# myscience/open-genie

Measured on NVIDIA B200. Metric: videotokenizer_train_step_frames_per_sec, higher is better.
Workload: dtype bf16

## Files before the change

open_genie_b200/csrc/conv3d_wgrad.cu:

```cuda
#include <stdlib.h>

#include "og_host.cuh"
#include "og_ptx.cuh"

namespace og {
extern std::atomic<uint64_t> g_launches;

struct WgradParams {
  int kt, kh, kw, pt, ph, pw;
  int ntaps, taps_per_group, num_groups, splitk;
  int block_n;
  int bw_log2, bh_log2, bt_log2, bn_log2;
  int tiles_w, tiles_h, tiles_t;
  int num_ksteps;
  int cin, cout;
  float* dw;
  long long ld_dw;
  int a_stages, b_stages;
  int sx_t, sx_h, sx_w;
  int vec_ok;
  float* dbias;
  int n_bias;
  int bias_col;
  int plain_store;
  int dbg;
};

static constexpr int kWThreads = 192;
static constexpr int kVox = 64;
static constexpr int kPanelBytes = kVox * 128;
static constexpr int kWABytes = 2 * kPanelBytes;
static constexpr int kWMaxStages = 12;

__global__ void __launch_bounds__(kWThreads, 1)
    og_conv_wgrad_kernel(const __grid_constant__ CUtensorMap mapDY, const __grid_constant__ CUtensorMap mapX,
                         const WgradParams p) {
  extern __shared__ uint8_t smem_raw[];
  uint8_t* smem = reinterpret_cast<uint8_t*>((reinterpret_cast<uintptr_t>(smem_raw) + 1023) & ~uintptr_t(1023));
  const int tap_bytes = (p.block_n / 64) * kPanelBytes;
  const int b_bytes = 2 * tap_bytes;
  uint8_t* smem_a = smem;
  uint8_t* smem_b = smem + p.a_stages * kWABytes;
  uint8_t* smem_ones = smem_b + p.b_stages * b_bytes;
  uint64_t* bars = reinterpret_cast<uint64_t*>(smem_ones + 2048);
  uint64_t* full_a = bars;
  uint64_t* empty_a = bars + kWMaxStages;
  uint64_t* full_b = bars + 2 * kWMaxStages;
  uint64_t* empty_b = bars + 3 * kWMaxStages;
  uint64_t* tmem_full = bars + 4 * kWMaxStages;
  uint32_t* tmem_slot = reinterpret_cast<uint32_t*>(bars + 4 * kWMaxStages + 1);

  const int warp = warp_idx_uniform();
  const int lane = threadIdx.x & 31;
  const int co0 = blockIdx.x * 128;
  const int ci0 = blockIdx.y * p.block_n;
  const int split = blockIdx.z / p.num_groups;
  const int group = blockIdx.z - split * p.num_groups;
  const int tap0 = group * p.taps_per_group;
  const int ntap = min(p.taps_per_group, p.ntaps - tap0);
  const bool do_bias = p.dbias != nullptr && blockIdx.y == 0 && group == p.num_groups - 1;
  const int ks_begin = (int)(((long long)p.num_ksteps * split) / p.splitk);
  const int ks_end = (int)(((long long)p.num_ksteps * (split + 1)) / p.splitk);

  if (warp == 0 && lane == 0) {
    tma_prefetch_desc(&mapDY);
    tma_prefetch_desc(&mapX);
    for (int s = 0; s < p.a_stages; ++s) {
      mbar_init(&full_a[s], 1);
      mbar_init(&empty_a[s], 1);
    }
    for (int s = 0; s < p.b_stages; ++s) {
      mbar_init(&full_b[s], 1);
      mbar_init(&empty_b[s], 1);
    }
    mbar_init(tmem_full, 1);
    fence_mbar_init();
  }
  if (warp == 1) tmem_alloc(tmem_slot, 512);
  if (do_bias) {
    for (int i = threadIdx.x; i < 2048 / 4; i += kWThreads) reinterpret_cast<uint32_t*>(smem_ones)[i] = 0x3F803F80u;
    fence_proxy_async_smem();
  }
  tc_fence_before();
  __syncthreads();
  tc_fence_after();
  const uint32_t tmem_base = *tmem_slot;

  if (warp == 0) {
    {
      int sa = 0, sb = 0;
      uint32_t pha = 0, phb = 0;
      int off_w[4], off_h[4], off_t[4];
#pragma unroll
      for (int j = 0; j < 4; ++j) {
        const int tap = tap0 + (j < ntap ? j : 0);
        off_t[j] = tap / (p.kh * p.kw) - p.pt;
        off_h[j] = (tap / p.kw) % p.kh - p.ph;
        off_w[j] = tap % p.kw - p.pw;
      }
      const int per_sample = p.tiles_w * p.tiles_h * p.tiles_t;
      int tn = ks_begin / per_sample;
      int r = ks_begin - tn * per_sample;
      int tw = r % p.tiles_w;
      r /= p.tiles_w;
      int th = r % p.tiles_h;
      int tt = r / p.tiles_h;
      const int panels = p.block_n / 64;
      for (int ks = ks_begin; ks < ks_end; ++ks) {
        const int n = tn << p.bn_log2, w0 = tw << p.bw_log2, h0 = th << p.bh_log2, t0 = tt << p.bt_log2;
        mbar_wait(&empty_a[sa], pha ^ 1);
        if (elect_one()) {
          mbar_expect_tx(&full_a[sa], kWABytes);
          tma_load_5d(smem_a + sa * kWABytes, &mapDY, &full_a[sa], co0, w0, h0, t0, n);
          tma_load_5d(smem_a + sa * kWABytes + kPanelBytes, &mapDY, &full_a[sa], co0 + 64, w0, h0, t0, n);
        }
        __syncwarp();
        if (++sa == p.a_stages) {
          sa = 0;
          pha ^= 1;
        }
#pragma unroll
        for (int j = 0; j < 4; j += 2) {
          if (j < ntap) {
            const int nt = (ntap - j) < 2 ? 1 : 2;
            mbar_wait(&empty_b[sb], phb ^ 1);
            if (elect_one()) {
              mbar_expect_tx(&full_b[sb], (uint32_t)(nt * tap_bytes));
              uint8_t* dst = smem_b + sb * b_bytes;
#pragma unroll
              for (int u = 0; u < 2; ++u) {
                if (u < nt) {
                  for (int pp = 0; pp < panels; ++pp)
                    tma_load_5d(dst + u * tap_bytes + pp * kPanelBytes, &mapX, &full_b[sb], ci0 + pp * 64,
                                w0 * p.sx_w + off_w[j + u], h0 * p.sx_h + off_h[j + u], t0 * p.sx_t + off_t[j + u], n);
                }
              }
            }
            __syncwarp();
            if (++sb == p.b_stages) {
              sb = 0;
              phb ^= 1;
            }
          }
        }
        if (++tw == p.tiles_w) {
          tw = 0;
          if (++th == p.tiles_h) {
            th = 0;
            if (++tt == p.tiles_t) {
              tt = 0;
              ++tn;
            }
          }
        }
      }
    }
    __syncwarp();
  } else if (warp == 1) {
    {
      const uint32_t amn = (p.dbg & 1) ? 0u : 1u, bmn = (p.dbg & 2) ? 0u : 1u;
      const uint32_t idesc1 = umma_idesc_bf16(128, (uint32_t)p.block_n, amn, bmn);
      const uint32_t idesc2 = umma_idesc_bf16(128, (uint32_t)(2 * p.block_n), amn, bmn);
      const uint32_t idesc_ones = umma_idesc_bf16(128, 16u, amn, 1u);
      int sa = 0, sb = 0;
      uint32_t pha = 0, phb = 0;
      for (int ks = ks_begin; ks < ks_end; ++ks) {
        mbar_wait(&full_a[sa], pha);
        tc_fence_after();
        const uint32_t a_addr = smem_u32(smem_a + sa * kWABytes);
        for (int j = 0; j < ntap; j += 2) {
          mbar_wait(&full_b[sb], phb);
          tc_fence_after();
          const uint32_t b_addr = smem_u32(smem_b + sb * b_bytes);
          const uint32_t d_tmem = tmem_base + j * p.block_n;
          const uint32_t idesc = (ntap - j >= 2) ? idesc2 : idesc1;
          if (elect_one()) {
#pragma unroll
            for (int k = 0; k < kVox / 16; ++k) {
              const uint64_t adesc = umma_smem_desc_sw128(a_addr + k * 2048, kPanelBytes, 1024);
              const uint64_t bdesc = umma_smem_desc_sw128(b_addr + k * 2048, kPanelBytes, 1024);
              umma_bf16_ss(d_tmem, adesc, bdesc, idesc, (ks > ks_begin || k > 0) ? 1u : 0u);
            }
            umma_commit(&empty_b[sb]);
          }
          __syncwarp();
          if (++sb == p.b_stages) {
            sb = 0;
            phb ^= 1;
          }
        }
        if (do_bias && elect_one()) {
          const uint32_t ones_addr = smem_u32(smem_ones);
#pragma unroll
          for (int k = 0; k < kVox / 16; ++k)
            umma_bf16_ss(tmem_base + p.bias_col, umma_smem_desc_sw128(a_addr + k * 2048, kPanelBytes, 1024),
                         umma_smem_desc_sw128(ones_addr, kPanelBytes, 1024), idesc_ones, (ks > ks_begin || k > 0) ? 1u : 0u);
        }
        __syncwarp();
        if (elect_one()) umma_commit(&empty_a[sa]);
        __syncwarp();
        if (++sa == p.a_stages) {
          sa = 0;
          pha ^= 1;
        }
      }
      if (elect_one()) umma_commit(tmem_full);
    }
    __syncwarp();
  } else {
    const int q = warp & 3;
    const int co = co0 + q * 32 + lane;
    if (p.dbg & 8)
      mbar_wait(tmem_full, 0);
    else
      mbar_wait_relaxed(tmem_full, 0);
    tc_fence_after();
    for (int j = 0; j < ntap && !(p.dbg & 4); ++j) {
      const int tap = tap0 + j;
      for (int c = 0; c < p.block_n; c += 32) {
        uint32_t v[32];
        tmem_ld_32x32(tmem_base + j * p.block_n + c + ((uint32_t)(q * 32) << 16), v);
        tmem_ld_wait();
        if (co < p.cout) {
          float* dst = p.dw + (long long)co * p.ld_dw + (long long)tap * p.cin + ci0 + c;
          if (p.vec_ok && ci0 + c + 32 <= p.cin && p.splitk == 1 && p.plain_store) {
#pragma unroll
            for (int jj = 0; jj < 32; jj += 4)
              *reinterpret_cast<float4*>(dst + jj) = make_float4(__uint_as_float(v[jj]), __uint_as_float(v[jj + 1]),
                                                                 __uint_as_float(v[jj + 2]), __uint_as_float(v[jj + 3]));
          } else if (p.vec_ok && ci0 + c + 32 <= p.cin) {
#pragma unroll
            for (int jj = 0; jj < 32; jj += 4)
              asm volatile("red.global.add.v4.f32 [%0], {%1, %2, %3, %4};" ::"l"(dst + jj), "f"(__uint_as_float(v[jj])),
                           "f"(__uint_as_float(v[jj + 1])), "f"(__uint_as_float(v[jj + 2])),
                           "f"(__uint_as_float(v[jj + 3]))
                           : "memory");
          } else {
#pragma unroll
            for (int jj = 0; jj < 32; ++jj)
              if (ci0 + c + jj < p.cin) atomicAdd(dst + jj, __uint_as_float(v[jj]));
          }
        }
      }
    }
    if (do_bias) {
      uint32_t v[16];
      tmem_ld_32x16(tmem_base + p.bias_col + ((uint32_t)(q * 32) << 16), v);
      tmem_ld_wait();
      if (co < p.n_bias) atomicAdd(p.dbias + co, __uint_as_float(v[0]));
    }
    tc_fence_before();
  }

  tc_fence_before();
  __syncthreads();
  if (warp == 1) {
    tc_fence_after();
    tmem_dealloc(tmem_base, 512);
  }
}

}

static int launch_wgrad(const void* dy, int cout, const void* x, int cin, float* dw, int64_t ld_dw, int kt, int kh, int kw,
                        int pt, int ph, int pw, int N, int T, int H, int W, int Ti, int Hi, int Wi, int st, int sh, int sw,
                        og_stream_t stream, float* dbias = nullptr, int n_bias = 0) {
  using namespace og;
  OG_REQUIRE(dy && x && dw, "conv3d_wgrad: null pointer");
  OG_REQUIRE(!dbias || (n_bias > 0 && n_bias <= cout), "conv3d_wgrad: n_bias=%d must be in 1..cout", n_bias);
  OG_REQUIRE(cin > 0 && cin % 64 == 0, "conv3d_wgrad: cin=%d must be a multiple of 64", cin);
  OG_REQUIRE(cout > 0 && cout % 8 == 0, "conv3d_wgrad: cout=%d must be a multiple of 8 (TMA row stride)", cout);
  OG_REQUIRE(kt >= 1 && kh >= 1 && kw >= 1 && pt >= 0 && ph >= 0 && pw >= 0 && pt < kt && ph < kh && pw < kw,
             "conv3d_wgrad: bad kernel/padding");
  OG_REQUIRE(st >= 1 && sh >= 1 && sw >= 1 && st <= 8 && sh <= 8 && sw <= 8, "conv3d_wgrad: bad stride");
  int bw, bh, bt, bn;
  choose_voxel_box(kVox, N, T, H, W, &bw, &bh, &bt, &bn);
  WgradParams p;
  memset(&p, 0, sizeof(p));
  p.kt = kt; p.kh = kh; p.kw = kw; p.pt = pt; p.ph = ph; p.pw = pw;
  p.sx_t = st; p.sx_h = sh; p.sx_w = sw;
  p.ntaps = kt * kh * kw;
  p.block_n = (cin % 128 == 0) ? 128 : 64;
  p.taps_per_group = 512 / p.block_n;
  if (p.taps_per_group > 4) p.taps_per_group = 4;
  if (p.taps_per_group > p.ntaps) p.taps_per_group = p.ntaps;
  p.num_groups = (p.ntaps + p.taps_per_group - 1) / p.taps_per_group;
  p.bw_log2 = ilog2(bw); p.bh_log2 = ilog2(bh); p.bt_log2 = ilog2(bt); p.bn_log2 = ilog2(bn);
  p.tiles_w = (W + bw - 1) / bw; p.tiles_h = (H + bh - 1) / bh; p.tiles_t = (T + bt - 1) / bt;
  p.num_ksteps = ((N + bn - 1) / bn) * p.tiles_w * p.tiles_h * p.tiles_t;
  p.cin = cin; p.cout = cout; p.dw = dw; p.ld_dw = ld_dw;
  const int co_tiles = (cout + 127) / 128;
  const int ci_tiles = cin / p.block_n;
  const int base_ctas = co_tiles * ci_tiles * p.num_groups;
  const int sms = num_sms();
  int max_split = p.num_ksteps / 4;
  if (max_split < 1) max_split = 1;
  if (max_split > 128) max_split = 128;
  int splitk = 1;
  double best = -1.0;
  for (int s = 1; s <= max_split; ++s) {
    const long long total = (long long)base_ctas * s;
    const long long waves = (total + sms - 1) / sms;
    if (waves > 3 && s > 1) break;
    const double eff = (double)total / (double)(waves * sms);
    if (eff > best + 1e-9) {
      best = eff;
      splitk = s;
    }
  }
  p.splitk = splitk;
  {
    const char* e = getenv("OG_WGRAD_DBG");
    p.dbg = e ? atoi(e) : 0;
    const char* ps = getenv("OG_WGRAD_PLAIN_STORE");
    p.plain_store = ps ? atoi(ps) : 0;
  }
  p.vec_ok = (ld_dw % 4 == 0) && (cin % 4 == 0) && ((reinterpret_cast<uintptr_t>(dw) & 15) == 0);
  bool colsum_after = false;
  if (dbias) {
    const int ntap_last = p.ntaps - (p.num_groups - 1) * p.taps_per_group;
    if (ntap_last * p.block_n + 16 <= 512 && !(p.dbg & 3)) {
      p.dbias = dbias;
      p.n_bias = n_bias;
      p.bias_col = ntap_last * p.block_n;
    } else {
      colsum_after = true;
    }
  }
  const int b_bytes = 2 * (p.block_n / 64) * kPanelBytes;
  p.a_stages = 3;
  p.b_stages = (int)((216 * 1024 - p.a_stages * kWABytes) / b_bytes);
  if (p.b_stages > kWMaxStages) p.b_stages = kWMaxStages;
  const size_t smem_bytes = (size_t)p.a_stages * kWABytes + (size_t)p.b_stages * b_bytes + 2048  + 1024 + 512;

  CUtensorMap mapDY, mapX;
  {
    uint64_t dims[5] = {(uint64_t)cout, (uint64_t)W, (uint64_t)H, (uint64_t)T, (uint64_t)N};
    uint64_t str[4] = {(uint64_t)cout * 2, (uint64_t)W * cout * 2, (uint64_t)H * W * cout * 2,
                       (uint64_t)T * H * W * cout * 2};
    uint32_t box[5] = {64, (uint32_t)bw, (uint32_t)bh, (uint32_t)bt, (uint32_t)bn};
    int r = make_tmap_bf16(&mapDY, dy, 5, dims, str, box);
    if (r != OG_OK) return r;
  }
  {
    uint64_t dims[5] = {(uint64_t)cin, (uint64_t)Wi, (uint64_t)Hi, (uint64_t)Ti, (uint64_t)N};
    uint64_t str[4] = {(uint64_t)cin * 2, (uint64_t)Wi * cin * 2, (uint64_t)Hi * Wi * cin * 2,
                       (uint64_t)Ti * Hi * Wi * cin * 2};
    uint32_t box[5] = {64, (uint32_t)(bw * sw), (uint32_t)(bh * sh), (uint32_t)(bt * st), (uint32_t)bn};
    uint32_t es[5] = {1, (uint32_t)sw, (uint32_t)sh, (uint32_t)st, 1};
    OG_REQUIRE(box[1] <= 256 && box[2] <= 256 && box[3] <= 256, "conv3d_wgrad: strided box exceeds the TMA limit");
    int r = make_tmap_bf16(&mapX, x, 5, dims, str, box, es);
    if (r != OG_OK) return r;
  }
  static bool attr_set = false;
  if (!attr_set) {
    OG_CHECK_CUDA(cudaFuncSetAttribute(og_conv_wgrad_kernel, cudaFuncAttributeMaxDynamicSharedMemorySize, 227 * 1024));
    attr_set = true;
  }
  dim3 grid(co_tiles, ci_tiles, p.num_groups * p.splitk);
  og_conv_wgrad_kernel<<<grid, kWThreads, smem_bytes, (cudaStream_t)stream>>>(mapDY, mapX, p);
  OG_CHECK_CUDA(cudaGetLastError());
  g_launches.fetch_add(1);
  if (colsum_after) return og_colsum(dy, (int64_t)N * T * H * W, n_bias, cout, dbias, stream);
  return OG_OK;
}

extern "C" int og_conv3d_wgrad(const void* dy, int cout, const void* x, int cin, float* dw, int64_t ld_dw, int kt,
                               int kh, int kw, int pt, int ph, int pw, int N, int T, int H, int W,
                               og_stream_t stream) {
  return launch_wgrad(dy, cout, x, cin, dw, ld_dw, kt, kh, kw, pt, ph, pw, N, T, H, W, T, H, W, 1, 1, 1, stream);
}

extern "C" int og_conv3d_wgrad_bias(const void* dy, int cout, const void* x, int cin, float* dw, int64_t ld_dw, int kt,
                                    int kh, int kw, int pt, int ph, int pw, int N, int T, int H, int W, float* dbias,
                                    int n_bias, og_stream_t stream) {
  if (!dbias) {
    og::set_error("conv3d_wgrad_bias: dbias is NULL");
    return OG_ERR_INVALID_ARGUMENT;
  }
  return launch_wgrad(dy, cout, x, cin, dw, ld_dw, kt, kh, kw, pt, ph, pw, N, T, H, W, T, H, W, 1, 1, 1, stream, dbias, n_bias);
}

extern "C" int og_conv3d_strided_wgrad(const void* dy, int cout, const void* x, int cin, float* dw, int64_t ld_dw, int kt,
                                       int kh, int kw, int st, int sh, int sw, int pt, int ph, int pw, int N, int T, int H,
                                       int W, og_stream_t stream) {
  const int To = (T + pt - kt) / st + 1, Ho = (H + 2 * ph - kh) / sh + 1, Wo = (W + 2 * pw - kw) / sw + 1;
  if (To < 1 || Ho < 1 || Wo < 1) {
    og::set_error("conv3d_strided_wgrad: empty output");
    return OG_ERR_INVALID_ARGUMENT;
  }
  return launch_wgrad(dy, cout, x, cin, dw, ld_dw, kt, kh, kw, pt, ph, pw, N, To, Ho, Wo, T, H, W, st, sh, sw, stream);
}
```

open_genie_b200/csrc/og_ptx.cuh:

```cuda
#pragma once
#include <cuda.h>
#include <cuda_bf16.h>
#include <cuda_runtime.h>
#include <stdint.h>

namespace og {

__device__ __forceinline__ uint32_t smem_u32(const void* p) {
  return static_cast<uint32_t>(__cvta_generic_to_shared(p));
}

__device__ __forceinline__ int warp_idx_uniform() { return __shfl_sync(0xffffffffu, (int)(threadIdx.x >> 5), 0); }
__device__ __forceinline__ bool elect_one() {
  uint32_t pred;
  asm volatile(
      "{\n"
      ".reg .pred P1;\n"
      "elect.sync _|P1, 0xffffffff;\n"
      "selp.u32 %0, 1, 0, P1;\n"
      "}\n"
      : "=r"(pred));
  return pred != 0;
}

__device__ __forceinline__ void mbar_init(uint64_t* bar, uint32_t count) {
  asm volatile("mbarrier.init.shared::cta.b64 [%0], %1;" ::"r"(smem_u32(bar)), "r"(count) : "memory");
}
__device__ __forceinline__ void fence_mbar_init() {
  asm volatile("fence.mbarrier_init.release.cluster;" ::: "memory");
}
__device__ __forceinline__ void fence_proxy_async_smem() {
  asm volatile("fence.proxy.async.shared::cta;" ::: "memory");
}
__device__ __forceinline__ void mbar_expect_tx(uint64_t* bar, uint32_t bytes) {
  asm volatile("mbarrier.arrive.expect_tx.shared::cta.b64 _, [%0], %1;" ::"r"(smem_u32(bar)), "r"(bytes)
               : "memory");
}
__device__ __forceinline__ void mbar_arrive(uint64_t* bar) {
  asm volatile("mbarrier.arrive.shared::cta.b64 _, [%0];" ::"r"(smem_u32(bar)) : "memory");
}
__device__ __forceinline__ bool mbar_try_wait(uint64_t* bar, uint32_t parity) {
  uint32_t ok;
  asm volatile(
      "{\n\t.reg .pred p;\n\t"
      "mbarrier.try_wait.parity.shared::cta.b64 p, [%1], %2;\n\t"
      "selp.u32 %0, 1, 0, p;\n\t}"
      : "=r"(ok)
      : "r"(smem_u32(bar)), "r"(parity)
      : "memory");
  return ok != 0;
}
#ifndef OG_MBAR_SPIN_LIMIT
#define OG_MBAR_SPIN_LIMIT (1u << 24)
#endif
__device__ __forceinline__ void mbar_wait(uint64_t* bar, uint32_t parity) {
  uint32_t spins = 0;
  while (!mbar_try_wait(bar, parity)) {
    if (++spins > OG_MBAR_SPIN_LIMIT) {
      printf("og: mbarrier wait timed out (block %d,%d,%d thread %d)\n", blockIdx.x, blockIdx.y, blockIdx.z,
             threadIdx.x);
      __trap();
    }
  }
}

__device__ __forceinline__ void mbar_wait_relaxed(uint64_t* bar, uint32_t parity) {
  uint32_t spins = 0;
  while (!mbar_try_wait(bar, parity)) {
    __nanosleep(spins < 64 ? 64 : 512);
    if (++spins > (OG_MBAR_SPIN_LIMIT >> 2)) {
      printf("og: mbarrier (relaxed) wait timed out (block %d,%d,%d thread %d)\n", blockIdx.x, blockIdx.y, blockIdx.z,
             threadIdx.x);
      __trap();
    }
  }
}

__device__ __forceinline__ void tma_prefetch_desc(const CUtensorMap* map) {
  asm volatile("prefetch.tensormap [%0];" ::"l"(map) : "memory");
}
__device__ __forceinline__ void tma_load_2d(void* smem, const CUtensorMap* map, uint64_t* bar, int c0, int c1) {
  asm volatile(
      "cp.async.bulk.tensor.2d.shared::cluster.global.mbarrier::complete_tx::bytes [%0], [%1, {%3, %4}], [%2];" ::"r"(
          smem_u32(smem)),
      "l"(map), "r"(smem_u32(bar)), "r"(c0), "r"(c1)
      : "memory");
}
__device__ __forceinline__ void tma_load_3d(void* smem, const CUtensorMap* map, uint64_t* bar, int c0, int c1, int c2) {
  asm volatile(
      "cp.async.bulk.tensor.3d.shared::cluster.global.mbarrier::complete_tx::bytes [%0], [%1, {%3, %4, %5}], "
      "[%2];" ::"r"(smem_u32(smem)),
      "l"(map), "r"(smem_u32(bar)), "r"(c0), "r"(c1), "r"(c2)
      : "memory");
}
__device__ __forceinline__ void tma_load_4d(void* smem, const CUtensorMap* map, uint64_t* bar, int c0, int c1, int c2,
                                            int c3) {
  asm volatile(
      "cp.async.bulk.tensor.4d.shared::cluster.global.mbarrier::complete_tx::bytes [%0], [%1, {%3, %4, %5, %6}], "
      "[%2];" ::"r"(smem_u32(smem)),
      "l"(map), "r"(smem_u32(bar)), "r"(c0), "r"(c1), "r"(c2), "r"(c3)
      : "memory");
}
__device__ __forceinline__ void tma_load_5d(void* smem, const CUtensorMap* map, uint64_t* bar, int c0, int c1, int c2,
                                            int c3, int c4) {
  asm volatile(
      "cp.async.bulk.tensor.5d.shared::cluster.global.mbarrier::complete_tx::bytes [%0], [%1, {%3, %4, %5, %6, %7}], "
      "[%2];" ::"r"(smem_u32(smem)),
      "l"(map), "r"(smem_u32(bar)), "r"(c0), "r"(c1), "r"(c2), "r"(c3), "r"(c4)
      : "memory");
}

__device__ __forceinline__ void tmem_alloc(uint32_t* smem_result, uint32_t ncols) {
  asm volatile("tcgen05.alloc.cta_group::1.sync.aligned.shared::cta.b32 [%0], %1;" ::"r"(smem_u32(smem_result)),
               "r"(ncols)
               : "memory");
  asm volatile("tcgen05.relinquish_alloc_permit.cta_group::1.sync.aligned;" ::: "memory");
}
__device__ __forceinline__ void tmem_dealloc(uint32_t taddr, uint32_t ncols) {
  asm volatile("tcgen05.dealloc.cta_group::1.sync.aligned.b32 %0, %1;" ::"r"(taddr), "r"(ncols) : "memory");
}
__device__ __forceinline__ void tc_fence_before() { asm volatile("tcgen05.fence::before_thread_sync;" ::: "memory"); }
__device__ __forceinline__ void tc_fence_after() { asm volatile("tcgen05.fence::after_thread_sync;" ::: "memory"); }

__device__ __forceinline__ void umma_bf16_ss(uint32_t tmem_d, uint64_t adesc, uint64_t bdesc, uint32_t idesc,
                                             uint32_t accumulate) {
  asm volatile(
      "{\n\t.reg .pred p;\n\t"
      "setp.ne.b32 p, %4, 0;\n\t"
      "tcgen05.mma.cta_group::1.kind::f16 [%0], %1, %2, %3, p;\n\t}" ::"r"(tmem_d),
      "l"(adesc), "l"(bdesc), "r"(idesc), "r"(accumulate)
      : "memory");
}
__device__ __forceinline__ void umma_commit(uint64_t* bar) {
  asm volatile("tcgen05.commit.cta_group::1.mbarrier::arrive::one.shared::cluster.b64 [%0];" ::"r"(smem_u32(bar))
               : "memory");
}
__device__ __forceinline__ void tmem_ld_wait() { asm volatile("tcgen05.wait::ld.sync.aligned;" ::: "memory"); }

__device__ __forceinline__ void tmem_ld_32x32(uint32_t taddr, uint32_t (&v)[32]) {
  asm volatile(
      "tcgen05.ld.sync.aligned.32x32b.x32.b32 "
      "{%0, %1, %2, %3, %4, %5, %6, %7, %8, %9, %10, %11, %12, %13, %14, %15, "
      "%16, %17, %18, %19, %20, %21, %22, %23, %24, %25, %26, %27, %28, %29, %30, %31}, [%32];"
      : "=r"(v[0]), "=r"(v[1]), "=r"(v[2]), "=r"(v[3]), "=r"(v[4]), "=r"(v[5]), "=r"(v[6]), "=r"(v[7]), "=r"(v[8]),
        "=r"(v[9]), "=r"(v[10]), "=r"(v[11]), "=r"(v[12]), "=r"(v[13]), "=r"(v[14]), "=r"(v[15]), "=r"(v[16]),
        "=r"(v[17]), "=r"(v[18]), "=r"(v[19]), "=r"(v[20]), "=r"(v[21]), "=r"(v[22]), "=r"(v[23]), "=r"(v[24]),
        "=r"(v[25]), "=r"(v[26]), "=r"(v[27]), "=r"(v[28]), "=r"(v[29]), "=r"(v[30]), "=r"(v[31])
      : "r"(taddr)
      : "memory");
}
__device__ __forceinline__ void tmem_st_32x32(uint32_t taddr, const uint32_t (&v)[32]) {
  asm volatile(
      "tcgen05.st.sync.aligned.32x32b.x32.b32 [%0], "
      "{%1, %2, %3, %4, %5, %6, %7, %8, %9, %10, %11, %12, %13, %14, %15, %16, "
      "%17, %18, %19, %20, %21, %22, %23, %24, %25, %26, %27, %28, %29, %30, %31, %32};" ::"r"(taddr),
      "r"(v[0]), "r"(v[1]), "r"(v[2]), "r"(v[3]), "r"(v[4]), "r"(v[5]), "r"(v[6]), "r"(v[7]), "r"(v[8]), "r"(v[9]),
      "r"(v[10]), "r"(v[11]), "r"(v[12]), "r"(v[13]), "r"(v[14]), "r"(v[15]), "r"(v[16]), "r"(v[17]), "r"(v[18]),
      "r"(v[19]), "r"(v[20]), "r"(v[21]), "r"(v[22]), "r"(v[23]), "r"(v[24]), "r"(v[25]), "r"(v[26]), "r"(v[27]),
      "r"(v[28]), "r"(v[29]), "r"(v[30]), "r"(v[31])
      : "memory");
}
__device__ __forceinline__ void tmem_st_wait() { asm volatile("tcgen05.wait::st.sync.aligned;" ::: "memory"); }
__device__ __forceinline__ float ex2_approx(float x) {
  float y;
  asm("ex2.approx.ftz.f32 %0, %1;" : "=f"(y) : "f"(x));
  return y;
}

__device__ __forceinline__ void tmem_ld_32x16(uint32_t taddr, uint32_t (&v)[16]) {
  asm volatile(
      "tcgen05.ld.sync.aligned.32x32b.x16.b32 "
      "{%0, %1, %2, %3, %4, %5, %6, %7, %8, %9, %10, %11, %12, %13, %14, %15}, [%16];"
      : "=r"(v[0]), "=r"(v[1]), "=r"(v[2]), "=r"(v[3]), "=r"(v[4]), "=r"(v[5]), "=r"(v[6]), "=r"(v[7]), "=r"(v[8]),
        "=r"(v[9]), "=r"(v[10]), "=r"(v[11]), "=r"(v[12]), "=r"(v[13]), "=r"(v[14]), "=r"(v[15])
      : "r"(taddr)
      : "memory");
}

__host__ __device__ __forceinline__ uint64_t umma_smem_desc_sw128(uint32_t smem_addr, uint32_t lbo_bytes,
                                                                  uint32_t sbo_bytes) {
  uint64_t d = 0;
  d |= static_cast<uint64_t>((smem_addr >> 4) & 0x3FFF);
  d |= static_cast<uint64_t>((lbo_bytes >> 4) & 0x3FFF) << 16;
  d |= static_cast<uint64_t>((sbo_bytes >> 4) & 0x3FFF) << 32;
  d |= static_cast<uint64_t>(1) << 46;
  d |= static_cast<uint64_t>(2) << 61;
  return d;
}
__host__ __device__ __forceinline__ uint32_t umma_idesc_bf16(uint32_t M, uint32_t N, uint32_t a_mn_major,
                                                             uint32_t b_mn_major) {
  return (1u << 4) | (1u << 7) | (1u << 10) | (a_mn_major << 15) | (b_mn_major << 16) | ((N >> 3) << 17) |
         ((M >> 4) << 24);
}

__device__ __forceinline__ uint32_t pack_bf16x2(float lo, float hi) {
  __nv_bfloat162 v = __floats2bfloat162_rn(lo, hi);
  return *reinterpret_cast<uint32_t*>(&v);
}

}
```

Baseline: 1967.

## Add 2-CTA paired UMMA wgrad path and cost-model tiling selection

Templates the conv3d weight-gradient kernel on a paired mode that uses cta_group::2 tcgen05 MMA with M=256 across a two-CTA cluster. In that mode each CTA loads half the X tap panels and signals the leader's barriers, which halves per-CTA B traffic and lets it use more A stages. The paired mode is opt-in through OG_WGRAD_PAIR. It also replaces the fixed taps-per-group and occupancy-only split-K heuristic with a cost model over bytes and MMA cycles per k-step, and this model is on by default. That can change grouping and split-K for every wgrad call, at the risk of picking worse configurations where the model's constants are off.

After: 1966 (median of 6 runs). Within noise of the previous version (-0.0%).

```diff
diff --git a/open_genie_b200/csrc/conv3d_wgrad.cu b/open_genie_b200/csrc/conv3d_wgrad.cu
--- a/open_genie_b200/csrc/conv3d_wgrad.cu
+++ b/open_genie_b200/csrc/conv3d_wgrad.cu
@@ -32,13 +32,15 @@
 static constexpr int kWABytes = 2 * kPanelBytes;
 static constexpr int kWMaxStages = 12;
 
+template <bool kPair>
 __global__ void __launch_bounds__(kWThreads, 1)
     og_conv_wgrad_kernel(const __grid_constant__ CUtensorMap mapDY, const __grid_constant__ CUtensorMap mapX,
                          const WgradParams p) {
   extern __shared__ uint8_t smem_raw[];
   uint8_t* smem = reinterpret_cast<uint8_t*>((reinterpret_cast<uintptr_t>(smem_raw) + 1023) & ~uintptr_t(1023));
   const int tap_bytes = (p.block_n / 64) * kPanelBytes;
-  const int b_bytes = 2 * tap_bytes;
+  const int b_bytes = kPair ? tap_bytes : 2 * tap_bytes;
+  const uint32_t rank = kPair ? cluster_ctarank() : 0u;
   uint8_t* smem_a = smem;
   uint8_t* smem_b = smem + p.a_stages * kWABytes;
   uint8_t* smem_ones = smem_b + p.b_stages * b_bytes;
@@ -76,13 +78,21 @@
     mbar_init(tmem_full, 1);
     fence_mbar_init();
   }
-  if (warp == 1) tmem_alloc(tmem_slot, 512);
+  if (warp == 1) {
+    if constexpr (kPair)
+      tmem_alloc_pair(tmem_slot, 512);
+    else
+      tmem_alloc(tmem_slot, 512);
+  }
   if (do_bias) {
     for (int i = threadIdx.x; i < 2048 / 4; i += kWThreads) reinterpret_cast<uint32_t*>(smem_ones)[i] = 0x3F803F80u;
     fence_proxy_async_smem();
   }
   tc_fence_before();
-  __syncthreads();
+  if constexpr (kPair)
+    cluster_sync();
+  else
+    __syncthreads();
   tc_fence_after();
   const uint32_t tmem_base = *tmem_slot;
 
@@ -110,9 +120,16 @@
         const int n = tn << p.bn_log2, w0 = tw << p.bw_log2, h0 = th << p.bh_log2, t0 = tt << p.bt_log2;
         mbar_wait(&empty_a[sa], pha ^ 1);
         if (elect_one()) {
-          mbar_expect_tx(&full_a[sa], kWABytes);
-          tma_load_5d(smem_a + sa * kWABytes, &mapDY, &full_a[sa], co0, w0, h0, t0, n);
-          tma_load_5d(smem_a + sa * kWABytes + kPanelBytes, &mapDY, &full_a[sa], co0 + 64, w0, h0, t0, n);
+          if constexpr (kPair) {
+            const uint32_t bar = mapa_shared(&full_a[sa], 0);
+            if (rank == 0) mbar_expect_tx(&full_a[sa], 2 * kWABytes);
+            tma_load_5d_pair(smem_a + sa * kWABytes, &mapDY, bar, co0, w0, h0, t0, n);
+            tma_load_5d_pair(smem_a + sa * kWABytes + kPanelBytes, &mapDY, bar, co0 + 64, w0, h0, t0, n);
+          } else {
+            mbar_expect_tx(&full_a[sa], kWABytes);
+            tma_load_5d(smem_a + sa * kWABytes, &mapDY, &full_a[sa], co0, w0, h0, t0, n);
+            tma_load_5d(smem_a + sa * kWABytes + kPanelBytes, &mapDY, &full_a[sa], co0 + 64, w0, h0, t0, n);
+          }
         }
         __syncwarp();
         if (++sa == p.a_stages) {
@@ -122,17 +139,28 @@
 #pragma unroll
         for (int j = 0; j < 4; j += 2) {
           if (j < ntap) {
-            const int nt = (ntap - j) < 2 ? 1 : 2;
+            const int nt = ((ntap - j) < 2 || (!kPair && (p.dbg & 16))) ? 1 : 2;
             mbar_wait(&empty_b[sb], phb ^ 1);
             if (elect_one()) {
-              mbar_expect_tx(&full_b[sb], (uint32_t)(nt * tap_bytes));
               uint8_t* dst = smem_b + sb * b_bytes;
-#pragma unroll
-              for (int u = 0; u < 2; ++u) {
-                if (u < nt) {
-                  for (int pp = 0; pp < panels; ++pp)
-                    tma_load_5d(dst + u * tap_bytes + pp * kPanelBytes, &mapX, &full_b[sb], ci0 + pp * 64,
-                                w0 * p.sx_w + off_w[j + u], h0 * p.sx_h + off_h[j + u], t0 * p.sx_t + off_t[j + u], n);
+              if constexpr (kPair) {
+                const int u = nt == 2 ? (int)rank : 0;
+                const int np = nt == 2 ? panels : 1;
+                const int pp0 = nt == 2 ? 0 : (int)rank;
+                if (rank == 0) mbar_expect_tx(&full_b[sb], (uint32_t)(2 * np * kPanelBytes));
+                const uint32_t bar = mapa_shared(&full_b[sb], 0);
+                for (int pp = 0; pp < np; ++pp)
+                  tma_load_5d_pair(dst + pp * kPanelBytes, &mapX, bar, ci0 + (pp0 + pp) * 64, w0 * p.sx_w + off_w[j + u],
+                                   h0 * p.sx_h + off_h[j + u], t0 * p.sx_t + off_t[j + u], n);
+              } else {
+                mbar_expect_tx(&full_b[sb], (uint32_t)(nt * tap_bytes));
+#pragma unroll
+                for (int u = 0; u < 2; ++u) {
+                  if (u < nt) {
+                    for (int pp = 0; pp < panels; ++pp)
+                      tma_load_5d(dst + u * tap_bytes + pp * kPanelBytes, &mapX, &full_b[sb], ci0 + pp * 64,
+                                  w0 * p.sx_w + off_w[j + u], h0 * p.sx_h + off_h[j + u], t0 * p.sx_t + off_t[j + u], n);
+                  }
                 }
               }
             }
@@ -157,11 +185,24 @@
     }
     __syncwarp();
   } else if (warp == 1) {
-    {
+    if (rank == 0) {
+      const uint32_t M = kPair ? 256u : 128u;
       const uint32_t amn = (p.dbg & 1) ? 0u : 1u, bmn = (p.dbg & 2) ? 0u : 1u;
-      const uint32_t idesc1 = umma_idesc_bf16(128, (uint32_t)p.block_n, amn, bmn);
-      const uint32_t idesc2 = umma_idesc_bf16(128, (uint32_t)(2 * p.block_n), amn, bmn);
-      const uint32_t idesc_ones = umma_idesc_bf16(128, 16u, amn, 1u);
+      const uint32_t idesc1 = umma_idesc_bf16(M, (uint32_t)p.block_n, amn, bmn);
+      const uint32_t idesc2 = umma_idesc_bf16(M, (uint32_t)(2 * p.block_n), amn, bmn);
+      const uint32_t idesc_ones = umma_idesc_bf16(M, 16u, amn, 1u);
+      auto mma = [](uint32_t d, uint64_t a, uint64_t b, uint32_t id, uint32_t acc) {
+        if constexpr (kPair)
+          umma_bf16_ss_pair(d, a, b, id, acc);
+        else
+          umma_bf16_ss(d, a, b, id, acc);
+      };
+      auto commit = [](uint64_t* bar) {
+        if constexpr (kPair)
+          umma_commit_pair(bar, 0x3);
+        else
+          umma_commit(bar);
+      };
       int sa = 0, sb = 0;
       uint32_t pha = 0, phb = 0;
       for (int ks = ks_begin; ks < ks_end; ++ks) {
@@ -179,9 +220,9 @@
             for (int k = 0; k < kVox / 16; ++k) {
               const uint64_t adesc = umma_smem_desc_sw128(a_addr + k * 2048, kPanelBytes, 1024);
               const uint64_t bdesc = umma_smem_desc_sw128(b_addr + k * 2048, kPanelBytes, 1024);
-              umma_bf16_ss(d_tmem, adesc, bdesc, idesc, (ks > ks_begin || k > 0) ? 1u : 0u);
+              mma(d_tmem, adesc, bdesc, idesc, (ks > ks_begin || k > 0) ? 1u : 0u);
             }
-            umma_commit(&empty_b[sb]);
+            commit(&empty_b[sb]);
           }
           __syncwarp();
           if (++sb == p.b_stages) {
@@ -193,18 +234,18 @@
           const uint32_t ones_addr = smem_u32(smem_ones);
 #pragma unroll
           for (int k = 0; k < kVox / 16; ++k)
-            umma_bf16_ss(tmem_base + p.bias_col, umma_smem_desc_sw128(a_addr + k * 2048, kPanelBytes, 1024),
+            mma(tmem_base + p.bias_col, umma_smem_desc_sw128(a_addr + k * 2048, kPanelBytes, 1024),
                          umma_smem_desc_sw128(ones_addr, kPanelBytes, 1024), idesc_ones, (ks > ks_begin || k > 0) ? 1u : 0u);
         }
         __syncwarp();
-        if (elect_one()) umma_commit(&empty_a[sa]);
+        if (elect_one()) commit(&empty_a[sa]);
         __syncwarp();
         if (++sa == p.a_stages) {
           sa = 0;
           pha ^= 1;
         }
       }
-      if (elect_one()) umma_commit(tmem_full);
+      if (elect_one()) commit(tmem_full);
     }
     __syncwarp();
   } else {
@@ -253,11 +294,94 @@
   }
 
   tc_fence_before();
-  __syncthreads();
+  if constexpr (kPair)
+    cluster_sync();
+  else
+    __syncthreads();
   if (warp == 1) {
     tc_fence_after();
-    tmem_dealloc(tmem_base, 512);
-  }
+    if constexpr (kPair)
+      tmem_dealloc_pair(tmem_base, 512);
+    else
+      tmem_dealloc(tmem_base, 512);
+  }
+}
+
+static void choose_wgrad_tiling(int tiling, bool pair, int ntaps, int block_n, int tiles, int num_ksteps, int sms,
+                                int* taps_per_group, int* splitk) {
+  int max_split = num_ksteps / 4;
+  if (max_split < 1) max_split = 1;
+  if (tiling == 0) {
+    int tpg = 512 / block_n;
+    if (tpg > 4) tpg = 4;
+    if (tpg > ntaps) tpg = ntaps;
+    const int base_ctas = tiles * ((ntaps + tpg - 1) / tpg);
+    if (max_split > 128) max_split = 128;
+    int best_s = 1;
+    double best = -1.0;
+    for (int s = 1; s <= max_split; ++s) {
+      const long long total = (long long)base_ctas * s;
+      const long long waves = (total + sms - 1) / sms;
+      if (waves > 3 && s > 1) break;
+      const double eff = (double)total / (double)(waves * sms);
+      if (eff > best + 1e-9) {
+        best = eff;
+        best_s = s;
+      }
+    }
+    *taps_per_group = tpg;
+    *splitk = best_s;
+    return;
+  }
+  const double kBytesPerClk = 60.0;
+  int best_tpg = 1, best_s = 1;
+  double best = 1e300;
+  const int tpg_min = ntaps < 2 ? ntaps : 2;
+  for (int tpg = 4; tpg >= tpg_min; --tpg) {
+    if (tpg > ntaps) continue;
+    const int groups = (ntaps + tpg - 1) / tpg;
+    const double x_bytes = tpg * block_n * (pair ? 64.0 : 128.0);
+    const double c_kstep = fmax(2.0 * block_n * tpg, (16384.0 + x_bytes) / kBytesPerClk);
+    const double c_fixed = 6000.0 + 64.0 * tpg * block_n;
+    for (int s = 1; s <= max_split; ++s) {
+      const long long total = (long long)tiles * groups * s;
+      const long long waves = (total + sms - 1) / sms;
+      if (waves > 3 && s > 1) break;
+      const double cost = (double)waves * ((double)((num_ksteps + s - 1) / s) * c_kstep + c_fixed);
+      if (cost < best * 0.97) {
+        best = cost;
+        best_tpg = tpg;
+        best_s = s;
+      }
+    }
+  }
+  *taps_per_group = best_tpg;
+  *splitk = best_s;
+}
+
+static int pair_slots() {
+  static int n = 0;
+  if (n == 0) {
+    cudaLaunchConfig_t cfg = {};
+    cfg.gridDim = dim3(2 * num_sms());
+    cfg.blockDim = dim3(kWThreads);
+    cfg.dynamicSmemBytes = 216 * 1024;
+    cudaLaunchAttribute attr[1];
+    attr[0].id = cudaLaunchAttributeClusterDimension;
+    attr[0].val.clusterDim.x = 2;
+    attr[0].val.clusterDim.y = 1;
+    attr[0].val.clusterDim.z = 1;
+    cfg.attrs = attr;
+    cfg.numAttrs = 1;
+    int c = 0;
+    cudaFuncSetAttribute(og_conv_wgrad_kernel<true>, cudaFuncAttributeMaxDynamicSharedMemorySize, 227 * 1024);
+    if (cudaOccupancyMaxActiveClusters(&c, og_conv_wgrad_kernel<true>, &cfg) != cudaSuccess || c <= 0) {
+      (void)cudaGetLastError();
+      c = num_sms() / 2;
+    }
+    n = c;
+  }
+  return n;
 }
 
 }
@@ -281,40 +405,27 @@
   p.sx_t = st; p.sx_h = sh; p.sx_w = sw;
   p.ntaps = kt * kh * kw;
   p.block_n = (cin % 128 == 0) ? 128 : 64;
-  p.taps_per_group = 512 / p.block_n;
-  if (p.taps_per_group > 4) p.taps_per_group = 4;
-  if (p.taps_per_group > p.ntaps) p.taps_per_group = p.ntaps;
-  p.num_groups = (p.ntaps + p.taps_per_group - 1) / p.taps_per_group;
   p.bw_log2 = ilog2(bw); p.bh_log2 = ilog2(bh); p.bt_log2 = ilog2(bt); p.bn_log2 = ilog2(bn);
   p.tiles_w = (W + bw - 1) / bw; p.tiles_h = (H + bh - 1) / bh; p.tiles_t = (T + bt - 1) / bt;
   p.num_ksteps = ((N + bn - 1) / bn) * p.tiles_w * p.tiles_h * p.tiles_t;
   p.cin = cin; p.cout = cout; p.dw = dw; p.ld_dw = ld_dw;
   const int co_tiles = (cout + 127) / 128;
   const int ci_tiles = cin / p.block_n;
-  const int base_ctas = co_tiles * ci_tiles * p.num_groups;
-  const int sms = num_sms();
-  int max_split = p.num_ksteps / 4;
-  if (max_split < 1) max_split = 1;
-  if (max_split > 128) max_split = 128;
-  int splitk = 1;
-  double best = -1.0;
-  for (int s = 1; s <= max_split; ++s) {
-    const long long total = (long long)base_ctas * s;
-    const long long waves = (total + sms - 1) / sms;
-    if (waves > 3 && s > 1) break;
-    const double eff = (double)total / (double)(waves * sms);
-    if (eff > best + 1e-9) {
-      best = eff;
-      splitk = s;
-    }
-  }
-  p.splitk = splitk;
+  bool pair = false;
   {
     const char* e = getenv("OG_WGRAD_DBG");
     p.dbg = e ? atoi(e) : 0;
     const char* ps = getenv("OG_WGRAD_PLAIN_STORE");
     p.plain_store = ps ? atoi(ps) : 0;
-  }
+    const char* tl = getenv("OG_WGRAD_TILING");
+    const int tiling = tl ? atoi(tl) : 1;
+    const char* pr = getenv("OG_WGRAD_PAIR");
+    pair = (pr ? atoi(pr) : 0) != 0 && co_tiles % 2 == 0 && p.block_n == 128 && !(p.dbg & 3);
+    const int sms = pair ? 2 * pair_slots() : num_sms();
+    choose_wgrad_tiling(tiling, pair, p.ntaps, p.block_n, co_tiles * ci_tiles, p.num_ksteps, sms, &p.taps_per_group,
+                        &p.splitk);
+  }
+  p.num_groups = (p.ntaps + p.taps_per_group - 1) / p.taps_per_group;
   p.vec_ok = (ld_dw % 4 == 0) && (cin % 4 == 0) && ((reinterpret_cast<uintptr_t>(dw) & 15) == 0);
   bool colsum_after = false;
   if (dbias) {
@@ -327,8 +438,14 @@
       colsum_after = true;
     }
   }
-  const int b_bytes = 2 * (p.block_n / 64) * kPanelBytes;
-  p.a_stages = 3;
+  const int b_bytes = (pair ? 1 : 2) * (p.block_n / 64) * kPanelBytes;
+  if (pair) {
+    const int b_per_kstep = p.taps_per_group >= 2 ? 2 : 1;
+    p.a_stages = (216 * 1024) / (kWABytes + b_per_kstep * b_bytes);
+    if (p.a_stages > kWMaxStages) p.a_stages = kWMaxStages;
+  } else {
+    p.a_stages = 3;
+  }
   p.b_stages = (int)((216 * 1024 - p.a_stages * kWABytes) / b_bytes);
   if (p.b_stages > kWMaxStages) p.b_stages = kWMaxStages;
   const size_t smem_bytes = (size_t)p.a_stages * kWABytes + (size_t)p.b_stages * b_bytes + 2048  + 1024 + 512;
@@ -354,11 +471,28 @@
   }
   static bool attr_set = false;
   if (!attr_set) {
-    OG_CHECK_CUDA(cudaFuncSetAttribute(og_conv_wgrad_kernel, cudaFuncAttributeMaxDynamicSharedMemorySize, 227 * 1024));
+    OG_CHECK_CUDA(cudaFuncSetAttribute(og_conv_wgrad_kernel<false>, cudaFuncAttributeMaxDynamicSharedMemorySize, 227 * 1024));
+    OG_CHECK_CUDA(cudaFuncSetAttribute(og_conv_wgrad_kernel<true>, cudaFuncAttributeMaxDynamicSharedMemorySize, 227 * 1024));
     attr_set = true;
   }
   dim3 grid(co_tiles, ci_tiles, p.num_groups * p.splitk);
-  og_conv_wgrad_kernel<<<grid, kWThreads, smem_bytes, (cudaStream_t)stream>>>(mapDY, mapX, p);
+  if (pair) {
+    cudaLaunchConfig_t cfg = {};
+    cfg.gridDim = grid;
+    cfg.blockDim = dim3(kWThreads);
+    cfg.dynamicSmemBytes = smem_bytes;
+    cfg.stream = (cudaStream_t)stream;
+    cudaLaunchAttribute attr[1];
+    attr[0].id = cudaLaunchAttributeClusterDimension;
+    attr[0].val.clusterDim.x = 2;
+    attr[0].val.clusterDim.y = 1;
+    attr[0].val.clusterDim.z = 1;
+    cfg.attrs = attr;
+    cfg.numAttrs = 1;
+    OG_CHECK_CUDA(cudaLaunchKernelEx(&cfg, og_conv_wgrad_kernel<true>, mapDY, mapX, p));
+  } else {
+    og_conv_wgrad_kernel<false><<<grid, kWThreads, smem_bytes, (cudaStream_t)stream>>>(mapDY, mapX, p);
+  }
   OG_CHECK_CUDA(cudaGetLastError());
   g_launches.fetch_add(1);
   if (colsum_after) return og_colsum(dy, (int64_t)N * T * H * W, n_bias, cout, dbias, stream);
diff --git a/open_genie_b200/csrc/og_ptx.cuh b/open_genie_b200/csrc/og_ptx.cuh
--- a/open_genie_b200/csrc/og_ptx.cuh
+++ b/open_genie_b200/csrc/og_ptx.cuh
@@ -110,6 +110,52 @@
       : "memory");
 }
 
+__device__ __forceinline__ uint32_t cluster_ctarank() {
+  uint32_t r;
+  asm volatile("mov.u32 %0, %%cluster_ctarank;" : "=r"(r));
+  return r;
+}
+__device__ __forceinline__ void cluster_sync() {
+  asm volatile("barrier.cluster.arrive.release.aligned;\n\tbarrier.cluster.wait.acquire.aligned;" ::: "memory");
+}
+__device__ __forceinline__ uint32_t mapa_shared(const void* p, uint32_t rank) {
+  uint32_t r;
+  asm volatile("mapa.shared::cluster.u32 %0, %1, %2;" : "=r"(r) : "r"(smem_u32(p)), "r"(rank));
+  return r;
+}
+__device__ __forceinline__ void tma_load_5d_pair(void* smem, const CUtensorMap* map, uint32_t bar_cluster, int c0, int c1,
+                                                 int c2, int c3, int c4) {
+  asm volatile(
+      "cp.async.bulk.tensor.5d.cta_group::2.shared::cluster.global.mbarrier::complete_tx::bytes [%0], [%1, {%3, %4, %5, %6, "
+      "%7}], [%2];" ::"r"(smem_u32(smem)),
+      "l"(map), "r"(bar_cluster), "r"(c0), "r"(c1), "r"(c2), "r"(c3), "r"(c4)
+      : "memory");
+}
+__device__ __forceinline__ void tmem_alloc_pair(uint32_t* smem_result, uint32_t ncols) {
+  asm volatile("tcgen05.alloc.cta_group::2.sync.aligned.shared::cta.b32 [%0], %1;" ::"r"(smem_u32(smem_result)),
+               "r"(ncols)
+               : "memory");
+  asm volatile("tcgen05.relinquish_alloc_permit.cta_group::2.sync.aligned;" ::: "memory");
+}
+__device__ __forceinline__ void tmem_dealloc_pair(uint32_t taddr, uint32_t ncols) {
+  asm volatile("tcgen05.dealloc.cta_group::2.sync.aligned.b32 %0, %1;" ::"r"(taddr), "r"(ncols) : "memory");
+}
+__device__ __forceinline__ void umma_bf16_ss_pair(uint32_t tmem_d, uint64_t adesc, uint64_t bdesc, uint32_t idesc,
+                                                  uint32_t accumulate) {
+  asm volatile(
+      "{\n\t.reg .pred p;\n\t"
+      "setp.ne.b32 p, %4, 0;\n\t"
+      "tcgen05.mma.cta_group::2.kind::f16 [%0], %1, %2, %3, p;\n\t}" ::"r"(tmem_d),
+      "l"(adesc), "l"(bdesc), "r"(idesc), "r"(accumulate)
+      : "memory");
+}
+__device__ __forceinline__ void umma_commit_pair(uint64_t* bar, uint16_t cta_mask) {
+  asm volatile("tcgen05.commit.cta_group::2.mbarrier::arrive::one.shared::cluster.multicast::cluster.b64 [%0], %1;" ::"r"(
+                   smem_u32(bar)),
+               "h"(cta_mask)
+               : "memory");
+}
+
 __device__ __forceinline__ void tmem_alloc(uint32_t* smem_result, uint32_t ncols) {
   asm volatile("tcgen05.alloc.cta_group::1.sync.aligned.shared::cta.b32 [%0], %1;" ::"r"(smem_u32(smem_result)),
                "r"(ncols)
```
